# Bergvca/string_grouper

Measured on AMD Instinct MI355X. Metric: hot-path rows/sec (the device path of match_strings: tokenise + tf-idf + postings + SpGEMM-topn, inputs resident in HBM), 663k-name self-join ntop=10 min_sim=0.8; match_strings end to end: match_strings_rows_per_s, higher is better.
Workload: dtype f32

## Files before the change

### string_grouper_amd/csrc/sg_vectorize.hip

```cpp
#include <memory>
#include <type_traits>

#include "sg_internal.h"

#define TOK_CAP 1024
#define SG_KEY_OOV32 0xFFFFFFFEu
#define SG_KEY_OOV64 0xFFFFFFFFFFFFFFFEull
#define SG_CHAR_ABSENT 0xFFFFu
#define TOK_CHARS (TOK_CAP + 16)

template <typename KeyT>
struct KeyTraits;
template <>
struct KeyTraits<uint32_t> {
    static constexpr uint32_t OOV = SG_KEY_OOV32;
    static constexpr uint32_t PAD = 0xFFFFFFFFu;
};
template <>
struct KeyTraits<uint64_t> {
    static constexpr uint64_t OOV = SG_KEY_OOV64;
    static constexpr uint64_t PAD = 0xFFFFFFFFFFFFFFFFull;
};

struct TokenCache {
// ... 323 lines not shown
                        keys[i + j] = a;
                    }
                }
                wave_sync();
            }
        }
        int uniq = 0;
        for (int base = 0; base < g; base += 64) {
            const int idx = base + lane;
            bool head = false;
            if (idx < g) head = (idx == 0) || (keys[idx] != keys[idx - 1]);
            const uint64_t hm = __ballot(head);
            if (head) starts[uniq + __popcll(hm & lt_mask)] = (uint16_t)idx;
            uniq += __popcll(hm);
        }
        if (lane == 0) starts[uniq] = (uint16_t)g;
        wave_sync();
        const int64_t obase = ub_ptr[row] - ub_ptr[0];
        for (int u = lane; u < uniq; u += 64) {
            const int s0 = starts[u];
            const KeyT key = keys[s0];
            out_keys[obase + u] = key;
            out_tf[obase + u] = (int32_t)starts[u + 1] - s0;
            if (df_table && key != KeyTraits<KeyT>::OOV) count_document(df_table, df_replicas, df_stride, row, (int64_t)key);
        }
        if (lane == 0) out_cnt[row] = uniq;
        wave_sync();
    }
}

template <typename KeyT, bool SYMBOLS>
__global__ void __launch_bounds__(256) tokenize_long_kernel(const void *__restrict__ chars_in,
                                                            const int64_t *__restrict__ offsets, TokParams p,
                                                            const uint32_t *__restrict__ long_rows,
                                                            const int64_t *__restrict__ coff, const int64_t *__restrict__ koff,
                                                            uint16_t *lchars, KeyT *lkeys,
                                                            const int64_t *__restrict__ ub_ptr, int32_t *__restrict__ out_cnt,
                                                            KeyT *__restrict__ out_keys, int32_t *__restrict__ out_tf,
                                                            int32_t *df_table, int32_t df_replicas, int64_t df_stride) {
    __shared__ int32_t wave_tot[4];
    __shared__ int32_t carry;
    const int tid = threadIdx.x, lane = tid & 63, wv = tid >> 6;
    const int64_t row = long_rows[blockIdx.x];
    const int64_t b0 = offsets[row];
    const int64_t len = offsets[row + 1] - b0;
    uint16_t *ch = lchars + coff[blockIdx.x];
    KeyT *keys = lkeys + koff[blockIdx.x];
    const int64_t P = koff[blockIdx.x + 1] - koff[blockIdx.x];
    if (tid == 0) carry = 0;
    __syncthreads();
    for (int64_t base = 0; base < len; base += 256) {
        uint32_t code = 0;
        const bool keep = base + tid < len && char_code<SYMBOLS>(chars_in, b0 + base + tid, p, &code);
        const uint64_t km = __ballot(keep);
        if (lane == 0) wave_tot[wv] = __popcll(km);
        __syncthreads();
        int before = carry;
        for (int w = 0; w < wv; ++w) before += wave_tot[w];
        if (keep) ch[before + __popcll(km & (((uint64_t)1 << lane) - 1))] = (uint16_t)code;
        __syncthreads();
        if (tid == 0) carry += wave_tot[0] + wave_tot[1] + wave_tot[2] + wave_tot[3];
        __syncthreads();
    }
    const int64_t m = carry;
    int64_t g = m - p.ngram + 1;
    if (g < 0) g = 0;
    for (int64_t idx = tid; idx < P; idx += 256) {
        KeyT key = KeyTraits<KeyT>::PAD;
        if (idx < g) {
            key = 0;
            bool absent = false;
            for (int q = 0; q < p.ngram; ++q) {
                const uint32_t c = ch[idx + q];
                absent |= c == SG_CHAR_ABSENT;
                key = (key << p.bits) | (KeyT)c;
            }
            if (absent) key = KeyTraits<KeyT>::OOV;
        }
        keys[idx] = key;
    }
    __syncthreads();
    for (int64_t k = 2; k <= P; k <<= 1) {
        for (int64_t j = k >> 1; j > 0; j >>= 1) {
            for (int64_t idx = tid; idx < (P >> 1); idx += 256) {
                const int64_t i = ((idx & ~(j - 1)) << 1) | (idx & (j - 1));
                const KeyT a = keys[i], b = keys[i + j];
                const bool up = (i & k) == 0;
                if ((a > b) == up) {
                    keys[i] = b;
                    keys[i + j] = a;
                }
            }
            __syncthreads();
        }
    }
    const int64_t obase = ub_ptr[row] - ub_ptr[0];
    __syncthreads();
    if (tid == 0) carry = 0;
    __syncthreads();
    for (int64_t base = 0; base < g; base += 256) {
        const int64_t idx = base + tid;
        const bool head = idx < g && (idx == 0 || keys[idx] != keys[idx - 1]);
        const uint64_t hm = __ballot(head);
        if (lane == 0) wave_tot[wv] = __popcll(hm);
        __syncthreads();
        int before = carry;
        for (int w = 0; w < wv; ++w) before += wave_tot[w];
        if (head) {
            const int64_t u = before + __popcll(hm & (((uint64_t)1 << lane) - 1));
            const KeyT key = keys[idx];
            int64_t e = idx + 1;
            while (e < g && keys[e] == key) ++e;
            out_keys[obase + u] = key;
            out_tf[obase + u] = (int32_t)(e - idx);
            if (df_table && key != KeyTraits<KeyT>::OOV) count_document(df_table, df_replicas, df_stride, row, (int64_t)key);
        }
        __syncthreads();
        if (tid == 0) carry += wave_tot[0] + wave_tot[1] + wave_tot[2] + wave_tot[3];
        __syncthreads();
    }
    if (tid == 0) out_cnt[row] = carry;
}

__global__ void __launch_bounds__(256) long_sizes_kernel(const int64_t *__restrict__ offsets, const uint32_t *__restrict__ long_rows,
                                                         uint32_t n_long, int64_t *sizes) {
    const uint32_t e = blockIdx.x * blockDim.x + threadIdx.x;
    if (e < n_long) sizes[e] = offsets[long_rows[e] + 1] - offsets[long_rows[e]];
}

__global__ void __launch_bounds__(256) df_reduce_kernel(int32_t *df_table, int64_t key_space, int32_t replicas, int64_t stride) {
    const int64_t i = (int64_t)blockIdx.x * blockDim.x + threadIdx.x;
    if (i >= key_space) return;
    int32_t s = df_table[i];
    for (int r = 1; r < replicas; ++r) s += df_table[(int64_t)r * stride + i];
    df_table[i] = s;
}

__global__ void __launch_bounds__(256) vocab_finalize_kernel(const int32_t *__restrict__ df_table, int64_t key_space,
                                                             int32_t *rank_io ,
                                                             uint64_t *col_keys, int32_t *col_df) {
    const int64_t i = (int64_t)blockIdx.x * blockDim.x + threadIdx.x;
    if (i >= key_space) return;
    const int32_t df = df_table[i];
    const int32_t r = rank_io[i];
    if (df > 0) {
        col_keys[r] = (uint64_t)i;
        col_df[r] = df;
    } else {
        rank_io[i] = -1;
    }
}


__global__ void __launch_bounds__(1024) df_count_lds_kernel(const int64_t *__restrict__ ub_ptr, const int32_t *__restrict__ cnt,
                                                            uint32_t *keys ,
                                                            const int32_t *__restrict__ key_to_col, int64_t n_rows,
                                                            int32_t col0, int32_t n_cols, int64_t n_terms,
                                                            uint32_t *__restrict__ partial,
                                                            int32_t cols_out ) {
    extern __shared__ uint32_t df_hist[];
    for (int k = threadIdx.x; k < n_cols; k += blockDim.x) df_hist[k] = 0;
    __syncthreads();
    const int64_t per_wg = (n_rows + gridDim.x - 1) / gridDim.x;
    const int64_t r0 = (int64_t)blockIdx.x * per_wg;
    int64_t r1 = r0 + per_wg;
    if (r1 > n_rows) r1 = n_rows;
    const int sub = threadIdx.x & 15;
    const int64_t groups = blockDim.x >> 4;
    for (int64_t rb = r0 + (threadIdx.x >> 4) * 4; rb < r1; rb += groups * 4) {
        int64_t b[4];
        int c[4];
#pragma unroll
        for (int r = 0; r < 4; ++r) {
            const bool valid = rb + r < r1;
            b[r] = valid ? ub_ptr[rb + r] - ub_ptr[0] : 0;
            c[r] = valid ? cnt[rb + r] : 0;
        }
        uint32_t key[4];
#pragma unroll
        for (int r = 0; r < 4; ++r) key[r] = sub < c[r] ? keys[b[r] + sub] : SG_KEY_OOV32;
        int32_t col[4];
#pragma unroll
        for (int r = 0; r < 4; ++r) col[r] = key[r] != SG_KEY_OOV32 ? key_to_col[key[r]] : -1;
#pragma unroll
        for (int r = 0; r < 4; ++r) {
            if (sub < c[r]) {
                if (cols_out) keys[b[r] + sub] = (uint32_t)col[r];
                const int32_t cc = col[r] - col0;
                if (col[r] >= 0 && cc >= 0 && cc < n_cols) atomicAdd(&df_hist[cc], 1u);
            }
            for (int q = sub + 16; q < c[r]; q += 16) {
                const uint32_t k2 = keys[b[r] + q];
                const int32_t c2 = k2 != SG_KEY_OOV32 ? key_to_col[k2] : -1;
                if (cols_out) keys[b[r] + q] = (uint32_t)c2;
                const int32_t cc = c2 - col0;
                if (c2 >= 0 && cc >= 0 && cc < n_cols) atomicAdd(&df_hist[cc], 1u);
            }
        }
    }
    __syncthreads();
    for (int k = threadIdx.x; k < n_cols; k += blockDim.x) partial[(int64_t)blockIdx.x * n_terms + col0 + k] = df_hist[k];
}

__global__ void __launch_bounds__(256) df_sum_kernel(const uint32_t *__restrict__ partial, int32_t n_partial, int64_t n_terms,
                                                     int32_t *__restrict__ df) {
    __shared__ uint32_t part[4][64];
    const int kk = threadIdx.x & 63, q = threadIdx.x >> 6;
    const int64_t k = (int64_t)blockIdx.x * 64 + kk;
    const int per = (n_partial + 3) / 4;
    const int r0 = q * per, r1 = r0 + per < n_partial ? r0 + per : n_partial;
    uint32_t s = 0;
    if (k < n_terms)
        for (int r = r0; r < r1; ++r) s += partial[(int64_t)r * n_terms + k];
    part[q][kk] = s;
    __syncthreads();
    if (q == 0 && k < n_terms) df[k] = (int32_t)(part[0][kk] + part[1][kk] + part[2][kk] + part[3][kk]);
}

struct DenseLookup {
    const int32_t *key_to_col;
    __device__ __forceinline__ int32_t operator()(uint32_t key) const { return key == SG_KEY_OOV32 ? -1 : key_to_col[key]; }
};
struct ColumnsLookup {
    __device__ __forceinline__ int32_t operator()(uint32_t key) const { return (int32_t)key; }
};
struct SortedLookup {
    const uint64_t *vocab;
    int64_t n_terms;
    __device__ __forceinline__ int32_t operator()(uint64_t key) const {
        int64_t lo = 0, hi = n_terms;
        while (lo < hi) {
            const int64_t mid = (lo + hi) >> 1;
            if (vocab[mid] < key) lo = mid + 1;
            else hi = mid;
        }
        return (lo < n_terms && vocab[lo] == key) ? (int32_t)lo : -1;
    }
};

template <typename KeyT, typename Lookup>
__global__ void __launch_bounds__(256) kept_count_kernel(const int64_t *__restrict__ ub_ptr,
                                                         const int32_t *__restrict__ cnt,
                                                         const KeyT *__restrict__ keys, Lookup lookup, int64_t n,
                                                         int32_t *kept) {
    const int64_t i = (int64_t)blockIdx.x * blockDim.x + threadIdx.x;
    if (i >= n) return;
    const int64_t b = ub_ptr[i] - ub_ptr[0];
    const int c = cnt[i];
    int k = 0;
    for (int q = 0; q < c; ++q) k += lookup(keys[b + q]) >= 0;
    kept[i] = k;
}

__global__ void __launch_bounds__(256) gather_keys_kernel(const int64_t *__restrict__ ub_ptr, const int32_t *__restrict__ cnt,
                                                          const uint64_t *__restrict__ keys, const int64_t *__restrict__ dst_ptr,
                                                          int64_t n, uint64_t *__restrict__ dst) {
    const int64_t i = (int64_t)blockIdx.x * blockDim.x + threadIdx.x;
    if (i >= n) return;
    const int64_t b = ub_ptr[i] - ub_ptr[0], d = dst_ptr[i];
    const int c = cnt[i];
    for (int q = 0; q < c; ++q) dst[d + q] = keys[b + q];
}

template <typename T>
__device__ __forceinline__ T tmul(T a, T b);
template <>
__device__ __forceinline__ float tmul<float>(float a, float b) { return __fmul_rn(a, b); }
template <>
__device__ __forceinline__ double tmul<double>(double a, double b) { return __dmul_rn(a, b); }

template <typename T, typename KeyT, typename Lookup>
__global__ void __launch_bounds__(256) weight_normalize_kernel(const int64_t *__restrict__ ub_ptr,
                                                               const int32_t *__restrict__ cnt,
                                                               const KeyT *__restrict__ keys,
                                                               const int32_t *__restrict__ tf, Lookup lookup,
                                                               const T *__restrict__ idf, int64_t n,
                                                               const int64_t *__restrict__ indptr,
                                                               int32_t *__restrict__ out_idx, T *__restrict__ out_val,
                                                               uint32_t *props ,
                                                               double *__restrict__ row_norm ) {
    const int64_t i = (int64_t)blockIdx.x * blockDim.x + threadIdx.x;
    float n2 = 0.f;
    uint32_t len = 0;
    if (i < n) {
        const int64_t b = ub_ptr[i] - ub_ptr[0];
        const int c = cnt[i];
        int64_t o = indptr[i];
        const int64_t o0 = o;
        double acc = 0.0;
        for (int q = 0; q < c; ++q) {
            const int32_t col = lookup(keys[b + q]);
            if (col < 0) continue;
            const T w = tmul<T>((T)tf[b + q], idf[col]);
            out_idx[o] = col;
            out_val[o] = w;
            acc = __dadd_rn(acc, (double)tmul<T>(w, w));
            ++o;
        }
        len = (uint32_t)(o - o0);
        const double nrm = acc != 0.0 ? __dsqrt_rn(acc) : 0.0;
        if (row_norm) row_norm[i] = nrm;
        if (acc != 0.0) {
            double s2 = 0.0;
            for (int64_t q = o0; q < o; ++q) {
                const T v = (T)__ddiv_rn((double)out_val[q], nrm);
                out_val[q] = v;
                s2 += (double)v * (double)v;
            }
            n2 = __double2float_ru(s2 * (1.0 + 1e-12));
        }
    }
    uint32_t nb = __float_as_uint(n2);
#pragma unroll
    for (int d = 32; d > 0; d >>= 1) {
        nb = max(nb, (uint32_t)__shfl_xor((int)nb, d, 64));
        len = max(len, (uint32_t)__shfl_xor((int)len, d, 64));
    }
    if ((threadIdx.x & 63) == 0 && props) {
        const volatile uint32_t *seen = props;
        if (nb > seen[1]) atomicMax(props + 1, nb);
        if (len > seen[2]) atomicMax(props + 2, len);
    }
}

__device__ __forceinline__ double dpp_from_lower_lane(double v, double lane0_gets) {
    const uint64_t b = (uint64_t)__double_as_longlong(v), o = (uint64_t)__double_as_longlong(lane0_gets);
    const uint32_t lo = (uint32_t)__builtin_amdgcn_update_dpp((int)(uint32_t)o, (int)(uint32_t)b, 0x111 , 0xF, 0xF, false);
    const uint32_t hi =
        (uint32_t)__builtin_amdgcn_update_dpp((int)(uint32_t)(o >> 32), (int)(uint32_t)(b >> 32), 0x111, 0xF, 0xF, false);
    return __longlong_as_double((long long)(((uint64_t)hi << 32) | lo));
}
__device__ __forceinline__ double shfl_double(double v, int src_lane) {
    const uint64_t b = (uint64_t)__double_as_longlong(v);
    const uint32_t lo = (uint32_t)__shfl((int)(uint32_t)b, src_lane, 64), hi = (uint32_t)__shfl((int)(uint32_t)(b >> 32), src_lane, 64);
    return __longlong_as_double((long long)(((uint64_t)hi << 32) | lo));
}

template <typename T, typename KeyT, typename Lookup>
__global__ void __launch_bounds__(256) weight_normalize_rows16_kernel(const int64_t *__restrict__ ub_ptr,
                                                                      const int32_t *__restrict__ cnt,
                                                                      const KeyT *__restrict__ keys,
                                                                      const int32_t *__restrict__ tf, Lookup lookup,
                                                                      const T *__restrict__ idf, int64_t n,
                                                                      const int64_t *__restrict__ indptr,
                                                                      int32_t *__restrict__ out_idx, T *__restrict__ out_val,
                                                                      uint32_t *props, double *__restrict__ row_norm) {
    const int lane = threadIdx.x & 63, sub = lane & 15, grp_shift = lane & 48;
    const int64_t row = ((int64_t)blockIdx.x * blockDim.x + threadIdx.x) >> 4;
    const bool valid = row < n;
    const int64_t b = valid ? ub_ptr[row] - ub_ptr[0] : 0;
    const int c = valid ? cnt[row] : 0;
    const int64_t o0 = valid ? indptr[row] : 0;
    int cmax = c;
    cmax = max(cmax, __shfl_xor(cmax, 16, 64));
    cmax = max(cmax, __shfl_xor(cmax, 32, 64));
    double carry = 0.0;
    int32_t col_keep[2] = {-1, -1};
    T w_keep[2] = {(T)0, (T)0};
    for (int base = 0; base < cmax; base += 16) {
        const int q = base + sub;
        double w2 = 0.0;
        if (q < c) {
            const int32_t col = lookup(keys[b + q]);
            if (col >= 0) {
                const T w = tmul<T>((T)tf[b + q], idf[col]);
                w2 = (double)tmul<T>(w, w);
                if (base == 0) {
                    col_keep[0] = col;
                    w_keep[0] = w;
                } else if (base == 16) {
                    col_keep[1] = col;
                    w_keep[1] = w;
                }
            }
        }
        double acc = w2;
#pragma unroll
        for (int k = 0; k < 16; ++k) acc = __dadd_rn(dpp_from_lower_lane(acc, carry), w2);
        carry = shfl_double(acc, lane | 15);
    }
    float n2 = 0.f;
    uint32_t len = 0;
    const double nrm = carry != 0.0 ? __dsqrt_rn(carry) : 0.0;
    if (valid && sub == 0 && row_norm) row_norm[row] = nrm;
    if (carry != 0.0) {
        double s2 = 0.0;
        int kept_before = 0;
        for (int base = 0; base < cmax; base += 16) {
            const int q = base + sub;
            int32_t col = -1;
            T w = 0;
            if (base < 32) {
                col = base == 0 ? col_keep[0] : col_keep[1];
                w = base == 0 ? w_keep[0] : w_keep[1];
            } else if (q < c) {
                col = lookup(keys[b + q]);
                if (col >= 0) w = tmul<T>((T)tf[b + q], idf[col]);
            }
            const uint32_t km = (uint32_t)(__ballot(col >= 0) >> grp_shift) & 0xFFFFu;
            if (col >= 0) {
                const int64_t o = o0 + kept_before + __popc(km & ((1u << sub) - 1u));
                const T v = (T)__ddiv_rn((double)w, nrm);
                out_idx[o] = col;
                out_val[o] = v;
                s2 += (double)v * (double)v;
            }
            kept_before += __popc(km);
        }
        len = (uint32_t)kept_before;
#pragma unroll
        for (int d = 8; d > 0; d >>= 1) s2 += shfl_double(s2, lane ^ d);
        n2 = __double2float_ru(s2 * (1.0 + 1e-12));
    }
    uint32_t nb = __float_as_uint(n2);
#pragma unroll
    for (int d = 32; d > 0; d >>= 1) {
        nb = max(nb, (uint32_t)__shfl_xor((int)nb, d, 64));
        len = max(len, (uint32_t)__shfl_xor((int)len, d, 64));
    }
    if (lane == 0 && props) {
        const volatile uint32_t *seen = props;
        if (nb > seen[1]) atomicMax(props + 1, nb);
        if (len > seen[2]) atomicMax(props + 2, len);
    }
}

__global__ void __launch_bounds__(1024) column_count_lds_kernel(const int64_t *__restrict__ indptr, int64_t n_rows,
                                                                const int32_t *__restrict__ indices, int32_t col0,
                                                                int32_t n_cols, int64_t n_terms,
                                                                uint32_t *__restrict__ partial) {
    extern __shared__ uint32_t df_hist[];
    for (int k = threadIdx.x; k < n_cols; k += blockDim.x) df_hist[k] = 0;
    __syncthreads();
    const int32_t *p = indices + indptr[0];
    const int64_t total = indptr[n_rows] - indptr[0];
    int64_t head = (int64_t)((0u - (uint32_t)((uintptr_t)p >> 2)) & 3u);
    if (head > total) head = total;
    const int64_t units = (total - head) >> 2;
    const int64_t tail0 = head + units * 4;
    const int4 *body = reinterpret_cast<const int4 *>(p + head);
    const int64_t per_wg = (units + gridDim.x - 1) / gridDim.x;
    const int64_t u0 = (int64_t)blockIdx.x * per_wg;
    int64_t u1 = u0 + per_wg;
    if (u1 > units) u1 = units;
    const uint32_t nc = (uint32_t)n_cols;
    for (int64_t u = u0 + threadIdx.x; u < u1; u += blockDim.x) {
        const int4 c = body[u];
        const uint32_t c0 = (uint32_t)(c.x - col0), c1 = (uint32_t)(c.y - col0), c2 = (uint32_t)(c.z - col0),
                       c3 = (uint32_t)(c.w - col0);
        if (c0 < nc) atomicAdd(&df_hist[c0], 1u);
        if (c1 < nc) atomicAdd(&df_hist[c1], 1u);
        if (c2 < nc) atomicAdd(&df_hist[c2], 1u);
        if (c3 < nc) atomicAdd(&df_hist[c3], 1u);
    }
    if (blockIdx.x == 0) {
        const int64_t e = (int64_t)threadIdx.x < head ? (int64_t)threadIdx.x : tail0 + ((int64_t)threadIdx.x - head);
        if (e < total) {
            const uint32_t c = (uint32_t)(p[e] - col0);
            if (c < nc) atomicAdd(&df_hist[c], 1u);
        }
    }
    __syncthreads();
    for (int k = threadIdx.x; k < n_cols; k += blockDim.x) partial[(int64_t)blockIdx.x * n_terms + col0 + k] = df_hist[k];
}

template <typename T>
struct ReweighEntry {
    int32_t col;
    T w;
    bool bad;
};
template <typename T>
__device__ __forceinline__ ReweighEntry<T> reweigh_entry(int32_t col, T v, double nrm_old, const T *__restrict__ idf_old,
                                                         const T *__restrict__ idf_new) {
    const T io = idf_old[col];
    const T tf = (T)rint(__ddiv_rn(__dmul_rn((double)v, nrm_old), (double)io));
    const T again = (T)__ddiv_rn((double)tmul<T>(tf, io), nrm_old);
    bool same;
    if (sizeof(T) == 4) same = __float_as_uint((float)again) == __float_as_uint((float)v);
    else same = __double_as_longlong((double)again) == __double_as_longlong((double)v);
    return ReweighEntry<T>{col, tmul<T>(tf, idf_new[col]), !same};
}

template <typename T>
__global__ void __launch_bounds__(256) reweigh_rows16_kernel(const int64_t *__restrict__ indptr,
                                                             const int32_t *__restrict__ in_idx, const T *__restrict__ in_val,
                                                             const double *__restrict__ in_norm, const T *__restrict__ idf_old,
                                                             const T *__restrict__ idf_new, int64_t n,
                                                             int64_t *__restrict__ out_indptr, int32_t *__restrict__ out_idx,
                                                             T *__restrict__ out_val, double *__restrict__ out_norm,
                                                             uint32_t *props, uint32_t *mismatch) {
    const int lane = threadIdx.x & 63, sub = lane & 15;
    const int64_t row = ((int64_t)blockIdx.x * blockDim.x + threadIdx.x) >> 4;
    const bool valid = row < n;
    const int64_t first = indptr[0];
    const int64_t b = valid ? indptr[row] : first;
    const int c = valid ? (int)(indptr[row + 1] - b) : 0;
    const int64_t o0 = b - first;
    const double nrm_old = valid ? in_norm[row] : 0.0;
    if (valid && sub == 0) {
        out_indptr[row] = o0;
        if (row == n - 1) out_indptr[n] = o0 + c;
    }
    int cmax = c;
    cmax = max(cmax, __shfl_xor(cmax, 16, 64));
    cmax = max(cmax, __shfl_xor(cmax, 32, 64));
    double carry = 0.0;
    int32_t col_keep[2] = {-1, -1};
    T w_keep[2] = {(T)0, (T)0};
    for (int base = 0; base < cmax; base += 16) {
        const int q = base + sub;
        double w2 = 0.0;
        if (q < c) {
            const ReweighEntry<T> e = reweigh_entry<T>(in_idx[b + q], in_val[b + q], nrm_old, idf_old, idf_new);
            if (e.bad) atomicAdd(mismatch, 1u);
            w2 = (double)tmul<T>(e.w, e.w);
            if (base == 0) {
                col_keep[0] = e.col;
                w_keep[0] = e.w;
            } else if (base == 16) {
                col_keep[1] = e.col;
                w_keep[1] = e.w;
            }
        }
        double acc = w2;
#pragma unroll
        for (int k = 0; k < 16; ++k) acc = __dadd_rn(dpp_from_lower_lane(acc, carry), w2);
        carry = shfl_double(acc, lane | 15);
    }
    float n2 = 0.f;
    uint32_t len = 0;
    const double nrm = carry != 0.0 ? __dsqrt_rn(carry) : 0.0;
    if (valid && sub == 0) out_norm[row] = nrm;
    if (carry != 0.0) {
        double s2 = 0.0;
        for (int base = 0; base < cmax; base += 16) {
            const int q = base + sub;
            if (q >= c) continue;
            int32_t col;
            T w;
            if (base < 32) {
                col = base == 0 ? col_keep[0] : col_keep[1];
                w = base == 0 ? w_keep[0] : w_keep[1];
            } else {
                const ReweighEntry<T> e = reweigh_entry<T>(in_idx[b + q], in_val[b + q], nrm_old, idf_old, idf_new);
                col = e.col;
                w = e.w;
            }
            const T v = (T)__ddiv_rn((double)w, nrm);
            out_idx[o0 + q] = col;
            out_val[o0 + q] = v;
            s2 += (double)v * (double)v;
        }
        len = (uint32_t)c;
#pragma unroll
        for (int d = 8; d > 0; d >>= 1) s2 += shfl_double(s2, lane ^ d);
        n2 = __double2float_ru(s2 * (1.0 + 1e-12));
    }
    uint32_t nb = __float_as_uint(n2);
#pragma unroll
    for (int d = 32; d > 0; d >>= 1) {
        nb = max(nb, (uint32_t)__shfl_xor((int)nb, d, 64));
        len = max(len, (uint32_t)__shfl_xor((int)len, d, 64));
    }
    if (lane == 0) {
// ... 489 lines not shown
    return SG_OK;
}

extern "C" int sg_vocab_coding(const sg_vocab *v, int32_t *bits_per_char, int32_t *symbols, int32_t *sorted_mode) {
    SG_REQUIRE(v && v->impl, "vocab is null");
    if (bits_per_char) *bits_per_char = v->bits_per_char;
    if (symbols) *symbols = v->impl->symbols ? 1 : 0;
    if (sorted_mode) *sorted_mode = v->sorted_mode ? 1 : 0;
    return SG_OK;
}

extern "C" int sg_vocab_to_host(sg_ctx *ctx, const sg_vocab *v, uint64_t *keys, int64_t *df) {
    SG_REQUIRE(ctx && v && keys && df, "null argument");
    const VocabImpl *im = impl_of(v);
    SG_REQUIRE(im != nullptr, "unknown vocab");
    std::vector<int32_t> hdf((size_t)v->n_terms);
    SG_HIP_TRY(hipMemcpyAsync(keys, v->d_keys, sizeof(uint64_t) * (size_t)v->n_terms, hipMemcpyDeviceToHost, ctx->stream));
    SG_HIP_TRY(hipMemcpyAsync(hdf.data(), v->d_df, sizeof(int32_t) * (size_t)v->n_terms, hipMemcpyDeviceToHost, ctx->stream));
    SG_HIP_TRY(hipStreamSynchronize(ctx->stream));
    for (int64_t i = 0; i < v->n_terms; ++i) df[i] = hdf[(size_t)i];
    return SG_OK;
}

extern "C" int sg_vocab_byte_alphabet(const sg_vocab *v, uint8_t *byte_of_code, int32_t *n_codes) {
    SG_REQUIRE(v && v->impl && byte_of_code && n_codes, "null argument");
    SG_REQUIRE(!v->impl->symbols, "the vocabulary was fitted on symbol columns: the caller holds their alphabet");
    *n_codes = 1 << v->bits_per_char;
    if (*n_codes > 128) *n_codes = 128;
    memcpy(byte_of_code, v->impl->byte_of_rank, (size_t)*n_codes);
    return SG_OK;
}

static bool weights_positive_and_finite(const void *w, int64_t n, int32_t dtype) {
    if (dtype == SG_F64) {
        const double *p = (const double *)w;
        for (int64_t i = 0; i < n; ++i)
            if (!(p[i] > 0.0) || !(p[i] <= 1.79e308)) return false;
    } else {
        const float *p = (const float *)w;
        for (int64_t i = 0; i < n; ++i)
            if (!(p[i] > 0.f) || !(p[i] <= 3.4e38f)) return false;
    }
    return true;
}

extern "C" int sg_vocab_set_idf(sg_ctx *ctx, sg_vocab *v, const void *idf, int32_t dtype) {
    SG_REQUIRE(ctx && v && idf, "null argument");
    SG_REQUIRE(dtype == v->params.dtype, "idf dtype differs from the vectoriser dtype");
    const size_t s = dtype == SG_F64 ? 8 : 4;
    v->idf_trusted = weights_positive_and_finite(idf, v->n_terms, dtype);
    if (!v->d_idf) SG_TRY(ctx->alloc(((size_t)v->n_terms + 1) * s, &v->d_idf));
    SG_HIP_TRY(hipMemcpyAsync(v->d_idf, idf, s * (size_t)v->n_terms, hipMemcpyHostToDevice, ctx->stream));
    SG_HIP_TRY(hipStreamSynchronize(ctx->stream));
    return SG_OK;
}

template <typename T>
__global__ void __launch_bounds__(256) idf_from_table_kernel(const int32_t *__restrict__ df, int64_t n_terms, const T *__restrict__ table,
                                                             int64_t n_docs, T *__restrict__ idf) {
    const int64_t k = (int64_t)blockIdx.x * blockDim.x + threadIdx.x;
    if (k >= n_terms) return;
    int64_t d = df[k];
    if (d < 0) d = 0;
    if (d > n_docs) d = n_docs;
    idf[k] = table[d];
}

extern "C" int sg_ctx_put_idf_table(sg_ctx *ctx, int64_t n_docs, int32_t dtype, const void *table) {
    SG_REQUIRE(ctx && table && n_docs >= 0, "null argument");
    SG_REQUIRE(dtype == SG_F32 || dtype == SG_F64, "dtype must be SG_F32 or SG_F64");
    const size_t bytes = ((size_t)n_docs + 1) * (dtype == SG_F64 ? 8 : 4);
    void *d = nullptr;
    SG_HIP_TRY(hipMalloc(&d, bytes));
    if (hipMemcpyAsync(d, table, bytes, hipMemcpyHostToDevice, ctx->stream) != hipSuccess ||
        hipStreamSynchronize(ctx->stream) != hipSuccess) {
        (void)hipFree(d);
        sg_set_error("upload of the idf table failed");
        return SG_ERR_HIP;
    }
    const bool trusted = weights_positive_and_finite((const char *)table + (dtype == SG_F64 ? 8 : 4), n_docs, dtype);
    for (auto &t : ctx->idf_tables)
        if (t.n_docs == n_docs && t.dtype == dtype) {
            (void)hipFree(t.d);
            t.d = d;
            t.trusted = trusted;
            return SG_OK;
        }
    if (ctx->idf_tables.size() >= 4) {
        (void)hipFree(ctx->idf_tables.front().d);
        ctx->idf_tables.erase(ctx->idf_tables.begin());
    }
    ctx->idf_tables.push_back({n_docs, dtype, d, trusted});
    return SG_OK;
}

extern "C" int sg_vocab_apply_idf_table(sg_ctx *ctx, sg_vocab *v, int32_t *applied) {
    SG_REQUIRE(ctx && v && applied, "null argument");
    *applied = 0;
    SG_REQUIRE(v->d_df != nullptr || v->n_terms == 0, "the vocabulary has no document counts (fit first)");
    const void *table = nullptr;
    bool trusted = false;
    for (const auto &t : ctx->idf_tables)
        if (t.n_docs == v->n_docs && t.dtype == v->params.dtype) {
            table = t.d;
            trusted = t.trusted;
        }
    if (!table) return SG_OK;
    v->idf_trusted = trusted;
    const size_t s = v->params.dtype == SG_F64 ? 8 : 4;
    if (!v->d_idf) SG_TRY(ctx->alloc(((size_t)v->n_terms + 1) * s, &v->d_idf));
    if (v->n_terms > 0) {
        const unsigned grid = (unsigned)((v->n_terms + 255) / 256);
        SG_TRY(by_dtype(v->params.dtype, [&](auto tag) -> int {
            using T = decltype(tag);
            hipLaunchKernelGGL(idf_from_table_kernel<T>, dim3(grid), dim3(256), 0, ctx->stream, (const int32_t *)v->d_df, v->n_terms,
                               (const T *)table, v->n_docs, (T *)v->d_idf);
            SG_HIP_TRY(hipGetLastError());
            return SG_OK;
        }));
    }
    *applied = 1;
    return SG_OK;
}

extern "C" int sg_vocab_free(sg_vocab *v) {
    if (!v) return SG_OK;
    VocabImpl *im = v->impl;
    v->impl = nullptr;
    sg_ctx *ctx = v->ctx;
    if (im) {
        for (auto &c : im->caches) free_cache(ctx, c);
        ctx->release(im->d_df_table);
        delete im;
    }
    ctx->release(v->d_key_to_col);
    ctx->release(v->d_keys);
    ctx->release(v->d_df);
    ctx->release(v->d_idf);
    delete v;
    return SG_OK;
}

template <typename KeyT, typename Lookup>
static int launch_weight(sg_ctx *ctx, const TokenCache &tc, Lookup lookup, const sg_vocab *v, const sg_csr *m) {
    const bool plain = ctx->opt_is("SG_K2_PLAIN", '1');
    return by_dtype(m->dtype, [&](auto tag) {
        using T = decltype(tag);
        if (plain)
            hipLaunchKernelGGL((weight_normalize_kernel<T, KeyT, Lookup>), dim3((unsigned)((m->n_rows + 255) / 256)), dim3(256), 0,
                               ctx->stream, (const int64_t *)tc.d_ub_ptr, (const int32_t *)tc.d_cnt, (const KeyT *)tc.d_keys,
                               (const int32_t *)tc.d_tf, lookup, (const T *)v->d_idf, m->n_rows, m->d_indptr,
                               (int32_t *)m->d_indices, (T *)m->d_data, m->d_props_words, m->d_row_norm);
        else
            hipLaunchKernelGGL((weight_normalize_rows16_kernel<T, KeyT, Lookup>), dim3((unsigned)((m->n_rows + 15) / 16)), dim3(256),
                               0, ctx->stream, (const int64_t *)tc.d_ub_ptr, (const int32_t *)tc.d_cnt, (const KeyT *)tc.d_keys,
                               (const int32_t *)tc.d_tf, lookup, (const T *)v->d_idf, m->n_rows, m->d_indptr,
                               (int32_t *)m->d_indices, (T *)m->d_data, m->d_props_words, m->d_row_norm);
        return hipGetLastError() == hipSuccess ? SG_OK : SG_ERR_HIP;
    });
}

struct RowPointers {
    int64_t *indptr = nullptr;
    int64_t nnz = 0;
};
static int row_pointers(sg_ctx *ctx, const sg_vocab *v, const TokenCache &tc, TokenCache *fitted, Scratch &tmp, RowPointers *out) {
    const int64_t n = tc.n;
    if (fitted && fitted->d_indptr && fitted->nnz >= 0 && n > 0) {
        *out = {fitted->d_indptr, fitted->nnz};
        fitted->d_indptr = nullptr;
        fitted->nnz = -1;
        return SG_OK;
    }
    int32_t *kept = nullptr;
    int64_t *indptr = nullptr;
    if (!fitted) SG_TRY(tmp.alloc((size_t)n + 1, &kept));
    SG_TRY(tmp.alloc((size_t)n + 1, &indptr));
    if (n == 0) {
        (void)hipMemsetAsync(indptr, 0, sizeof(int64_t), ctx->stream);
    } else if (fitted) {
        SG_TRY(sg_exclusive_scan_i32_to_i64(ctx, tc.d_cnt, indptr, n));
    } else {
        const unsigned grid = (unsigned)((n + 255) / 256);
        if (v->sorted_mode)
            hipLaunchKernelGGL((kept_count_kernel<uint64_t, SortedLookup>), dim3(grid), dim3(256), 0, ctx->stream,
                               (const int64_t *)tc.d_ub_ptr, (const int32_t *)tc.d_cnt, (const uint64_t *)tc.d_keys,
                               SortedLookup{v->d_keys, v->n_terms}, n, kept);
        else
            hipLaunchKernelGGL((kept_count_kernel<uint32_t, DenseLookup>), dim3(grid), dim3(256), 0, ctx->stream,
                               (const int64_t *)tc.d_ub_ptr, (const int32_t *)tc.d_cnt, (const uint32_t *)tc.d_keys,
                               DenseLookup{v->d_key_to_col}, n, kept);
        SG_TRY(sg_exclusive_scan_i32_to_i64(ctx, kept, indptr, n));
    }
    if (hipMemcpyAsync(&out->nnz, indptr + n, sizeof(int64_t), hipMemcpyDeviceToHost, ctx->stream) != hipSuccess ||
        hipStreamSynchronize(ctx->stream) != hipSuccess)
        return SG_ERR_HIP;
    out->indptr = tmp.keep(indptr);
    return SG_OK;
}

extern "C" int sg_vec_transform(sg_ctx *ctx, const sg_vocab *v, const sg_strings *strings, sg_csr **out) {
    SG_REQUIRE(ctx && v && strings && out, "null argument");
    SG_REQUIRE(v->d_idf != nullptr, "sg_vocab_set_idf has not been called");
    VocabImpl *im = impl_of(v);
    SG_REQUIRE(im != nullptr, "unknown vocab");
    SG_REQUIRE((strings->sym_width == 2) == im->symbols && (!im->symbols || strings->alphabet == im->alphabet),
               "the strings are not of the kind (bytes / symbols of this alphabet) the vocabulary was fitted on");
    CsrPtr m(new (std::nothrow) sg_csr());
    if (!m) return SG_ERR_OOM;
    m->ctx = ctx;
    m->n_rows = strings->n;
    m->n_cols = v->n_terms;
    m->dtype = v->params.dtype;
    m->owned = true;
    m->from_vectoriser = v->idf_trusted;
    OwnedTokens local(ctx);
    Scratch tmp(ctx);
    TokenCache *fitted = nullptr;
    for (auto &c : im->caches)
        if (c.src == strings && c.n == strings->n) fitted = &c;
    if (!fitted) {
        SgTimer timer(ctx, SG_K_TOKENIZE);
        SG_TRY(tokenize_set(ctx, v, strings, nullptr, 1, 0, &local.c));
    }
    const TokenCache &tc = fitted ? *fitted : local.c;
    SgTimer timer(ctx, SG_K_WEIGHT);
    RowPointers rp;
    SG_TRY(row_pointers(ctx, v, tc, fitted, tmp, &rp));
    m->d_indptr = rp.indptr;
    m->nnz = rp.nnz;
    int32_t *idx = nullptr;
    void *val = nullptr;
    SG_TRY(sg_alloc(ctx, (size_t)m->nnz + 4, &idx));
    m->d_indices = idx;
    SG_TRY(ctx->alloc(((size_t)m->nnz + 4) * (m->dtype == SG_F64 ? 8 : 4), &val));
    m->d_data = val;
    if (ctx->opt_is("SG_ROW_BLOCKS", '1')) {
        SG_TRY(sg_alloc(ctx, (size_t)4, &m->d_props_words));
        if (hipMemsetAsync(m->d_props_words, 0, 16, ctx->stream) != hipSuccess) return SG_ERR_HIP;
    }
    SG_TRY(sg_alloc(ctx, (size_t)m->n_rows + 1, &m->d_row_norm));
    if (m->n_rows > 0) {
        if (v->sorted_mode)
            SG_TRY(launch_weight<uint64_t>(ctx, tc, SortedLookup{v->d_keys, v->n_terms}, v, m.get()));
        else if (tc.keys_are_columns)
            SG_TRY(launch_weight<uint32_t>(ctx, tc, ColumnsLookup{}, v, m.get()));
        else
            SG_TRY(launch_weight<uint32_t>(ctx, tc, DenseLookup{v->d_key_to_col}, v, m.get()));
    }
    *out = m.release();
    return SG_OK;
}

static int column_counts_device(sg_ctx *ctx, const sg_csr *m, int32_t *d_counts) {
    const int32_t max_cols = 30 * 1024;
    SG_TRY(allow_dynamic_lds<column_count_lds_kernel>((size_t)max_cols * 4));
    int64_t g = (m->nnz + 16383) / 16384;
    g = std::max<int64_t>(1, std::min<int64_t>(g, ctx->num_cu));
    Scratch tmp(ctx);
    uint32_t *partial = nullptr;
    SG_TRY(tmp.alloc((size_t)(g * m->n_cols), &partial));
    for (int64_t col0 = 0; col0 < m->n_cols; col0 += max_cols) {
        const int32_t n_cols = (int32_t)std::min<int64_t>(m->n_cols - col0, max_cols);
        hipLaunchKernelGGL(column_count_lds_kernel, dim3((unsigned)g), dim3(1024), (size_t)n_cols * 4, ctx->stream, m->d_indptr,
                           m->n_rows, m->d_indices, (int32_t)col0, n_cols, m->n_cols, partial);
    }
    hipLaunchKernelGGL(df_sum_kernel, dim3((unsigned)((m->n_cols + 63) / 64)), dim3(256), 0, ctx->stream, (const uint32_t *)partial,
                       (int32_t)g, m->n_cols, d_counts);
    SG_HIP_TRY(hipGetLastError());
    return SG_OK;
}

extern "C" int sg_csr_column_counts(sg_ctx *ctx, const sg_csr *m, int32_t *counts_host) {
    SG_REQUIRE(ctx && m, "null argument");
    if (m->n_cols == 0) return SG_OK;
    SG_REQUIRE(counts_host != nullptr, "the counts' array is null");
    if (m->rows_of) SG_TRY(sg_csr_ensure_rows(ctx, m));
    Scratch tmp(ctx);
    int32_t *d_counts = nullptr;
    SG_TRY(tmp.alloc((size_t)m->n_cols, &d_counts));
    SG_TRY(column_counts_device(ctx, m, d_counts));
    return sg_fetch(ctx, counts_host, d_counts, sizeof(int32_t) * (size_t)m->n_cols);
}

extern "C" int sg_vec_reweigh(sg_ctx *ctx, sg_vocab *v, const sg_csr *m, const int32_t *df_host, int64_t n_docs,
                              const void *idf_host, int32_t dtype, sg_csr **out) {
    SG_REQUIRE(ctx && v && m && df_host && idf_host && out, "null argument");
    SG_REQUIRE(v->d_idf != nullptr && v->d_df != nullptr, "the vocabulary has no idf yet (sg_vocab_set_idf)");
    SG_REQUIRE(m->d_row_norm != nullptr, "the matrix carries no row norms: only what sg_vec_transform made can be weighted anew");
    SG_REQUIRE(m->n_cols == v->n_terms, "the matrix's columns are not the vocabulary's");
    SG_REQUIRE(dtype == v->params.dtype && dtype == m->dtype, "dtype differs from the vectoriser's or the matrix's");
    SG_REQUIRE(n_docs >= 0, "negative number of documents");
    SG_REQUIRE(weights_positive_and_finite(idf_host, v->n_terms, dtype), "an idf that is not positive and finite");
    const size_t s = dtype == SG_F64 ? 8 : 4;
    CsrPtr r(new (std::nothrow) sg_csr());
    if (!r) return SG_ERR_OOM;
    r->ctx = ctx;
    r->n_rows = m->n_rows;
    r->n_cols = m->n_cols;
    r->nnz = m->nnz;
    r->dtype = dtype;
    r->owned = true;
    r->from_vectoriser = true;
    int64_t *dp = nullptr;
    int32_t *di = nullptr;
    void *dd = nullptr;
    SG_TRY(sg_alloc(ctx, (size_t)r->n_rows + 1, &dp));
// ... 45 lines not shown
```

Measured before the change: 109.3 million.

## Software-pipeline df counting loads and process two rows per lane group in weighting

The df histogram kernel now runs a two-stage software pipeline: row metadata for the group after next and first keys for the next group are loaded while the current group's column lookups and LDS atomics are issued. It also preloads two keys per row instead of one. The weight/normalize kernel now handles SG_K2_ROWS (default 2) rows per 16-lane group, interleaving their loads and DPP prefix scans to raise memory-level parallelism, with half as many blocks launched. The cost is higher register pressure and lower occupancy.

```diff
diff --git a/string_grouper_amd/csrc/sg_vectorize.hip b/string_grouper_amd/csrc/sg_vectorize.hip
--- a/string_grouper_amd/csrc/sg_vectorize.hip
+++ b/string_grouper_amd/csrc/sg_vectorize.hip
@@ -499,6 +499,63 @@
 }
 
 
+struct DfTrip {
+    int64_t b[4];
+    int c[4];
+    uint32_t key[4][2];
+    int32_t col[4][2];
+    __device__ __forceinline__ void rows(const int64_t *__restrict__ ub_ptr, const int32_t *__restrict__ cnt, int64_t ub0, int64_t rb,
+                                         int64_t r1) {
+#pragma unroll
+        for (int r = 0; r < 4; ++r) {
+            const bool valid = rb + r < r1;
+            b[r] = valid ? ub_ptr[rb + r] : ub0;
+            c[r] = valid ? cnt[rb + r] : 0;
+        }
+    }
+    __device__ __forceinline__ void take_rows(const DfTrip &o) {
+#pragma unroll
+        for (int r = 0; r < 4; ++r) {
+            b[r] = o.b[r];
+            c[r] = o.c[r];
+        }
+    }
+    __device__ __forceinline__ void first_keys(const uint32_t *keys, int64_t ub0, int sub) {
+#pragma unroll
+        for (int r = 0; r < 4; ++r) b[r] -= ub0;
+#pragma unroll
+        for (int r = 0; r < 4; ++r)
+#pragma unroll
+            for (int h = 0; h < 2; ++h) key[r][h] = sub + 16 * h < c[r] ? keys[b[r] + sub + 16 * h] : SG_KEY_OOV32;
+    }
+    __device__ __forceinline__ void columns(const int32_t *__restrict__ key_to_col) {
+#pragma unroll
+        for (int r = 0; r < 4; ++r)
+#pragma unroll
+            for (int h = 0; h < 2; ++h) col[r][h] = key[r][h] != SG_KEY_OOV32 ? key_to_col[key[r][h]] : -1;
+    }
+    __device__ __forceinline__ void count(uint32_t *keys, const int32_t *__restrict__ key_to_col, int sub, int32_t col0, int32_t n_cols,
+                                          int32_t cols_out, uint32_t *df_hist) const {
+#pragma unroll
+        for (int r = 0; r < 4; ++r) {
+#pragma unroll
+            for (int h = 0; h < 2; ++h)
+                if (sub + 16 * h < c[r]) {
+                    if (cols_out) keys[b[r] + sub + 16 * h] = (uint32_t)col[r][h];
+                    const int32_t cc = col[r][h] - col0;
+                    if (col[r][h] >= 0 && cc >= 0 && cc < n_cols) atomicAdd(&df_hist[cc], 1u);
+                }
+            for (int q = sub + 32; q < c[r]; q += 16) {
+                const uint32_t k2 = keys[b[r] + q];
+                const int32_t c2 = k2 != SG_KEY_OOV32 ? key_to_col[k2] : -1;
+                if (cols_out) keys[b[r] + q] = (uint32_t)c2;
+                const int32_t cc = c2 - col0;
+                if (c2 >= 0 && cc >= 0 && cc < n_cols) atomicAdd(&df_hist[cc], 1u);
+            }
+        }
+    }
+};
+
 __global__ void __launch_bounds__(1024) df_count_lds_kernel(const int64_t *__restrict__ ub_ptr, const int32_t *__restrict__ cnt,
                                                             uint32_t *keys ,
                                                             const int32_t *__restrict__ key_to_col, int64_t n_rows,
@@ -514,36 +571,27 @@
     if (r1 > n_rows) r1 = n_rows;
     const int sub = threadIdx.x & 15;
     const int64_t groups = blockDim.x >> 4;
-    for (int64_t rb = r0 + (threadIdx.x >> 4) * 4; rb < r1; rb += groups * 4) {
-        int64_t b[4];
-        int c[4];
-#pragma unroll
-        for (int r = 0; r < 4; ++r) {
-            const bool valid = rb + r < r1;
-            b[r] = valid ? ub_ptr[rb + r] - ub_ptr[0] : 0;
-            c[r] = valid ? cnt[rb + r] : 0;
-        }
-        uint32_t key[4];
-#pragma unroll
-        for (int r = 0; r < 4; ++r) key[r] = sub < c[r] ? keys[b[r] + sub] : SG_KEY_OOV32;
-        int32_t col[4];
-#pragma unroll
-        for (int r = 0; r < 4; ++r) col[r] = key[r] != SG_KEY_OOV32 ? key_to_col[key[r]] : -1;
-#pragma unroll
-        for (int r = 0; r < 4; ++r) {
-            if (sub < c[r]) {
-                if (cols_out) keys[b[r] + sub] = (uint32_t)col[r];
-                const int32_t cc = col[r] - col0;
-                if (col[r] >= 0 && cc >= 0 && cc < n_cols) atomicAdd(&df_hist[cc], 1u);
-            }
-            for (int q = sub + 16; q < c[r]; q += 16) {
-                const uint32_t k2 = keys[b[r] + q];
-                const int32_t c2 = k2 != SG_KEY_OOV32 ? key_to_col[k2] : -1;
-                if (cols_out) keys[b[r] + q] = (uint32_t)c2;
-                const int32_t cc = c2 - col0;
-                if (c2 >= 0 && cc >= 0 && cc < n_cols) atomicAdd(&df_hist[cc], 1u);
-            }
-        }
+    const int64_t ub0 = ub_ptr[0];
+    const int64_t step = groups * 4;
+    int64_t rb = r0 + (threadIdx.x >> 4) * 4;
+    DfTrip X, Y, ahead;
+    X.rows(ub_ptr, cnt, ub0, rb, r1);
+    Y.rows(ub_ptr, cnt, ub0, rb + step, r1);
+    X.first_keys(keys, ub0, sub);
+    while (rb < r1) {
+        X.columns(key_to_col);
+        Y.first_keys(keys, ub0, sub);
+        ahead.rows(ub_ptr, cnt, ub0, rb + 2 * step, r1);
+        X.count(keys, key_to_col, sub, col0, n_cols, cols_out, df_hist);
+        rb += step;
+        if (rb >= r1) break;
+        X.take_rows(ahead);
+        Y.columns(key_to_col);
+        X.first_keys(keys, ub0, sub);
+        ahead.rows(ub_ptr, cnt, ub0, rb + 2 * step, r1);
+        Y.count(keys, key_to_col, sub, col0, n_cols, cols_out, df_hist);
+        rb += step;
+        Y.take_rows(ahead);
     }
     __syncthreads();
     for (int k = threadIdx.x; k < n_cols; k += blockDim.x) partial[(int64_t)blockIdx.x * n_terms + col0 + k] = df_hist[k];
@@ -683,6 +731,9 @@
     return __longlong_as_double((long long)(((uint64_t)hi << 32) | lo));
 }
 
+#ifndef SG_K2_ROWS
+#define SG_K2_ROWS 2
+#endif
 template <typename T, typename KeyT, typename Lookup>
 __global__ void __launch_bounds__(256) weight_normalize_rows16_kernel(const int64_t *__restrict__ ub_ptr,
                                                                       const int32_t *__restrict__ cnt,
@@ -692,72 +743,120 @@
                                                                       const int64_t *__restrict__ indptr,
                                                                       int32_t *__restrict__ out_idx, T *__restrict__ out_val,
                                                                       uint32_t *props, double *__restrict__ row_norm) {
+    constexpr int R = SG_K2_ROWS;
     const int lane = threadIdx.x & 63, sub = lane & 15, grp_shift = lane & 48;
-    const int64_t row = ((int64_t)blockIdx.x * blockDim.x + threadIdx.x) >> 4;
-    const bool valid = row < n;
-    const int64_t b = valid ? ub_ptr[row] - ub_ptr[0] : 0;
-    const int c = valid ? cnt[row] : 0;
-    const int64_t o0 = valid ? indptr[row] : 0;
-    int cmax = c;
+    const int64_t row0 = (((int64_t)blockIdx.x * blockDim.x + threadIdx.x) >> 4) * R;
+    const int64_t ub0 = ub_ptr[0];
+    bool valid[R];
+    int64_t b[R], o0[R];
+    int c[R];
+#pragma unroll
+    for (int i = 0; i < R; ++i) {
+        valid[i] = row0 + i < n;
+        b[i] = valid[i] ? ub_ptr[row0 + i] : ub0;
+        c[i] = valid[i] ? cnt[row0 + i] : 0;
+        o0[i] = valid[i] ? indptr[row0 + i] : 0;
+    }
+    int cmax = 0;
+#pragma unroll
+    for (int i = 0; i < R; ++i) {
+        b[i] -= ub0;
+        cmax = max(cmax, c[i]);
+    }
     cmax = max(cmax, __shfl_xor(cmax, 16, 64));
     cmax = max(cmax, __shfl_xor(cmax, 32, 64));
-    double carry = 0.0;
-    int32_t col_keep[2] = {-1, -1};
-    T w_keep[2] = {(T)0, (T)0};
+    double carry[R];
+    int32_t col_keep[R][2];
+    T w_keep[R][2];
+#pragma unroll
+    for (int i = 0; i < R; ++i) {
+        carry[i] = 0.0;
+        col_keep[i][0] = col_keep[i][1] = -1;
+        w_keep[i][0] = w_keep[i][1] = (T)0;
+    }
     for (int base = 0; base < cmax; base += 16) {
         const int q = base + sub;
-        double w2 = 0.0;
-        if (q < c) {
-            const int32_t col = lookup(keys[b + q]);
-            if (col >= 0) {
-                const T w = tmul<T>((T)tf[b + q], idf[col]);
-                w2 = (double)tmul<T>(w, w);
+        KeyT key[R];
+        int32_t t[R], col[R];
+        T f[R];
+#pragma unroll
+        for (int i = 0; i < R; ++i) {
+            key[i] = q < c[i] ? keys[b[i] + q] : (KeyT)0;
+            t[i] = q < c[i] ? tf[b[i] + q] : 0;
+        }
+#pragma unroll
+        for (int i = 0; i < R; ++i) col[i] = q < c[i] ? lookup(key[i]) : -1;
+#pragma unroll
+        for (int i = 0; i < R; ++i) f[i] = col[i] >= 0 ? idf[col[i]] : (T)0;
+        double w2[R], acc[R];
+#pragma unroll
+        for (int i = 0; i < R; ++i) {
+            w2[i] = 0.0;
+            if (col[i] >= 0) {
+                const T w = tmul<T>((T)t[i], f[i]);
+                w2[i] = (double)tmul<T>(w, w);
                 if (base == 0) {
-                    col_keep[0] = col;
-                    w_keep[0] = w;
+                    col_keep[i][0] = col[i];
+                    w_keep[i][0] = w;
                 } else if (base == 16) {
-                    col_keep[1] = col;
-                    w_keep[1] = w;
+                    col_keep[i][1] = col[i];
+                    w_keep[i][1] = w;
                 }
             }
-        }
-        double acc = w2;
-#pragma unroll
-        for (int k = 0; k < 16; ++k) acc = __dadd_rn(dpp_from_lower_lane(acc, carry), w2);
-        carry = shfl_double(acc, lane | 15);
+            acc[i] = w2[i];
+        }
+#pragma unroll
+        for (int k = 0; k < 16; ++k) {
+#pragma unroll
+            for (int i = 0; i < R; ++i) acc[i] = __dadd_rn(dpp_from_lower_lane(acc[i], carry[i]), w2[i]);
+        }
+#pragma unroll
+        for (int i = 0; i < R; ++i) carry[i] = shfl_double(acc[i], lane | 15);
     }
     float n2 = 0.f;
     uint32_t len = 0;
-    const double nrm = carry != 0.0 ? __dsqrt_rn(carry) : 0.0;
-    if (valid && sub == 0 && row_norm) row_norm[row] = nrm;
-    if (carry != 0.0) {
-        double s2 = 0.0;
-        int kept_before = 0;
-        for (int base = 0; base < cmax; base += 16) {
-            const int q = base + sub;
+    double nrm[R], s2[R];
+    int kept_before[R];
+#pragma unroll
+    for (int i = 0; i < R; ++i) {
+        nrm[i] = carry[i] != 0.0 ? __dsqrt_rn(carry[i]) : 0.0;
+        if (valid[i] && sub == 0 && row_norm) row_norm[row0 + i] = nrm[i];
+        s2[i] = 0.0;
+        kept_before[i] = 0;
+    }
+    for (int base = 0; base < cmax; base += 16) {
+        const int q = base + sub;
+#pragma unroll
+        for (int i = 0; i < R; ++i) {
+            if (carry[i] == 0.0) continue;
             int32_t col = -1;
             T w = 0;
             if (base < 32) {
-                col = base == 0 ? col_keep[0] : col_keep[1];
-                w = base == 0 ? w_keep[0] : w_keep[1];
-            } else if (q < c) {
-                col = lookup(keys[b + q]);
-                if (col >= 0) w = tmul<T>((T)tf[b + q], idf[col]);
+                col = base == 0 ? col_keep[i][0] : col_keep[i][1];
+                w = base == 0 ? w_keep[i][0] : w_keep[i][1];
+            } else if (q < c[i]) {
+                col = lookup(keys[b[i] + q]);
+                if (col >= 0) w = tmul<T>((T)tf[b[i] + q], idf[col]);
             }
             const uint32_t km = (uint32_t)(__ballot(col >= 0) >> grp_shift) & 0xFFFFu;
             if (col >= 0) {
-                const int64_t o = o0 + kept_before + __popc(km & ((1u << sub) - 1u));
-                const T v = (T)__ddiv_rn((double)w, nrm);
+                const int64_t o = o0[i] + kept_before[i] + __popc(km & ((1u << sub) - 1u));
+                const T v = (T)__ddiv_rn((double)w, nrm[i]);
                 out_idx[o] = col;
                 out_val[o] = v;
-                s2 += (double)v * (double)v;
-            }
-            kept_before += __popc(km);
-        }
-        len = (uint32_t)kept_before;
-#pragma unroll
-        for (int d = 8; d > 0; d >>= 1) s2 += shfl_double(s2, lane ^ d);
-        n2 = __double2float_ru(s2 * (1.0 + 1e-12));
+                s2[i] += (double)v * (double)v;
+            }
+            kept_before[i] += __popc(km);
+        }
+    }
+#pragma unroll
+    for (int i = 0; i < R; ++i) {
+        if (carry[i] == 0.0) continue;
+        len = max(len, (uint32_t)kept_before[i]);
+        double s = s2[i];
+#pragma unroll
+        for (int d = 8; d > 0; d >>= 1) s += shfl_double(s, lane ^ d);
+        n2 = fmaxf(n2, __double2float_ru(s * (1.0 + 1e-12)));
     }
     uint32_t nb = __float_as_uint(n2);
 #pragma unroll
@@ -1553,7 +1652,8 @@
                                (const int32_t *)tc.d_tf, lookup, (const T *)v->d_idf, m->n_rows, m->d_indptr,
                                (int32_t *)m->d_indices, (T *)m->d_data, m->d_props_words, m->d_row_norm);
         else
-            hipLaunchKernelGGL((weight_normalize_rows16_kernel<T, KeyT, Lookup>), dim3((unsigned)((m->n_rows + 15) / 16)), dim3(256),
+            hipLaunchKernelGGL((weight_normalize_rows16_kernel<T, KeyT, Lookup>),
+                               dim3((unsigned)((m->n_rows + 16 * SG_K2_ROWS - 1) / (16 * SG_K2_ROWS))), dim3(256),
                                0, ctx->stream, (const int64_t *)tc.d_ub_ptr, (const int32_t *)tc.d_cnt, (const KeyT *)tc.d_keys,
                                (const int32_t *)tc.d_tf, lookup, (const T *)v->d_idf, m->n_rows, m->d_indptr,
                                (int32_t *)m->d_indices, (T *)m->d_data, m->d_props_words, m->d_row_norm);
```

Measured after the change: 109.5 million (median of 3 runs). About the same (+0.2%).
